# soopark0221/auction-gym

Measured on AMD Instinct MI355X. Metric: auctions resolved/sec (SP_Oracle-shaped batches), higher is better.
Workload: dtype f64

## Files before the change

### auction-gym_amd/csrc/ag_host.h

```cpp
#pragma once
#include <hip/hip_runtime.h>
#include <stdint.h>

#include "auctiongym.h"

int ag_set_error(int code, const char *fmt, ...) __attribute__((format(printf, 2, 3)));

#define AG_HIP(call)                                                                    \
  do {                                                                                  \
    hipError_t e_ = (call);                                                             \
    if (e_ != hipSuccess)                                                               \
      return ag_set_error(AG_ERR_HIP, "%s: %s (%s:%d)", #call, hipGetErrorString(e_),   \
                          __FILE__, __LINE__);                                          \
  } while (0)

template <typename T>
inline int ag_check_struct(const T *p, const char *who, const char *type) {
  if (p && p->struct_size != (uint64_t)sizeof(T))
    return ag_set_error(AG_ERR_INVALID,
                        "%s: %s.struct_size is %llu, this library (ABI %d) expects %llu -- the caller's "
                        "binding declares another layout of include/auctiongym.h",
                        who, type, (unsigned long long)p->struct_size, AG_ABI_VERSION,
                        (unsigned long long)sizeof(T));
  return AG_OK;
// ... 32 lines not shown
  uint32_t *key = nullptr;
  float *x = nullptr;
  int64_t *offsets = nullptr;
  double *adam_tab = nullptr;
  int32_t *epochs = nullptr;
  void *tables = nullptr;
  int64_t *partials = nullptr;
  size_t tables_bytes = 0, partials_bytes = 0;
  int coop_blocks = 0;
  struct {
    bool active = false;
    void *st = nullptr;
    void *acc = nullptr, *tables = nullptr;
    size_t st_bytes = 0, acc_bytes = 0, tables_bytes = 0;
    agtrain::RpAcc A{};
    agtrain::RpTables T{};
    int G = 0;
    int64_t k = 0;
    int64_t *totals = nullptr;
  } rp;
};

struct ag_dr_rp {
  bool active = false;
  void *st = nullptr;
  void *acc = nullptr, *tables = nullptr;
  size_t st_bytes = 0, acc_bytes = 0, tables_bytes = 0;
  agtrain::RpAcc A{};
  agtrain::RpTables T{};
  int G = 0, lines = 0;
  int64_t k = 0;
  int64_t *totals = nullptr;
  const float *noise = nullptr;
  int64_t noise_n = 0;
  int32_t noise_e0 = 0, noise_epochs = 0;
  agtrain::SortedRecs recs{};
  bool single = false;
  void *pipe = nullptr;
  size_t pipe_bytes = 0;
  void *pipe_st = nullptr;
  int pipe_blocks[2] = {0, 0};
};

struct ag_dr_ws {
  void *buf = nullptr;
  size_t buf_bytes = 0;
  int64_t *counts = nullptr;
  double *adam_tab = nullptr;
  float *state = nullptr;
  int32_t *init = nullptr;
  int32_t *mode = nullptr;
  int64_t *scratch = nullptr;
  void *coop = nullptr;
  size_t coop_bytes = 0;
  int coop_blocks = 0;
  int coop_blocks0 = 0;
  ag_dr_rp rp;
};

struct ag_ctx {
  int32_t device;
  ag_shape shape;
  int32_t D;
  int32_t item_search = AG_ITEM_SEARCH_AUTO;
  bool can_simulate = false;
  double *d_items = nullptr;
  double *d_values = nullptr;
  int64_t *d_partials = nullptr;
  uint32_t *d_queue = nullptr;
  int32_t partial_blocks = 0;
  int32_t resident[256] = {};
  bool ship_shape = true;
  bool gen_mode_all = false;
  int64_t launch_cap = 0;
  int64_t lrts_chunk = 0;
  bool wide = false;
  bool catalog = false;
  bool values_positive = false;
  bool ora_catalog = false;
  int32_t sim_kernel = AG_SIM_KERNEL_AUTO;
  int32_t grid_per_cu = 0;
  int32_t block_threads = 0;
  int32_t resident_slots[3][8] = {};
  int32_t resident_ora[8] = {};
  bool general = false, has_lrts = false, has_shading = false, lrts_loaded = false;
  int32_t ts_sample = 1;
  int32_t *h_akind = nullptr;
  int32_t *h_bkind = nullptr;
  bool dr_loaded = false, dr_any_init = false;
  bool vl_any_search = false;
  int64_t bidder_chunk = 0;
  int64_t bidder_cache = -1;
  uint64_t fit_noise_seed = 0;
  ag_dr_ws dr;
  int32_t *d_akind = nullptr, *d_bkind = nullptr;
  int32_t *d_kag = nullptr;
  bool ragged = false;
  double *d_pg = nullptr, *d_gs = nullptr;
  float *d_tsm = nullptr, *d_tsq = nullptr, *d_tsprev = nullptr;
  ag_lrts_ws lrts;
  int32_t *d_status = nullptr;
};

void ag_lrts_release(ag_ctx *c);
void ag_dr_release(ag_ctx *c);

inline int ag_one_slot_only(const ag_ctx *c, const char *who) {
  if (c && c->shape.num_slots > 1)
    return ag_set_error(AG_ERR_UNSUPPORTED, "%s: the context has num_slots = %d; rounds with several slots run "
                        "through ag_simulate_slots", who, c->shape.num_slots);
  return AG_OK;
}

inline int ag_check_store(const ag_ctx *c, const ag_lrts_samples *s, const char *who) {
  if (!c || !s) return ag_set_error(AG_ERR_INVALID, "%s: null argument", who);
  AG_CHECK_STRUCT(s, who, "ag_lrts_samples");
  if (!s->key || !s->x || !s->count || s->capacity < 0)
    return ag_set_error(AG_ERR_INVALID, "%s: sample store needs key, x, count and capacity >= 0", who);
  return AG_OK;
}
inline int ag_check_store(const ag_ctx *c, const ag_shading_samples *s, const char *who) {
  if (!c || !s) return ag_set_error(AG_ERR_INVALID, "%s: null argument", who);
  AG_CHECK_STRUCT(s, who, "ag_shading_samples");
  if (!s->agent || !s->gamma || !s->utility || !s->count || s->capacity < 0)
    return ag_set_error(AG_ERR_INVALID, "%s: sample store needs agent, gamma, utility, count, capacity", who);
  return AG_OK;
}

struct AgDeviceGuard {
  int prev = -1;
  explicit AgDeviceGuard(int dev) {
    if (hipGetDevice(&prev) == hipSuccess && prev != dev) (void)hipSetDevice(dev);
    else prev = -1;
  }
  ~AgDeviceGuard() {
    if (prev >= 0) (void)hipSetDevice(prev);
  }
};
```

### auction-gym_amd/csrc/ag_kernels.hip

```cpp
#include <hip/hip_runtime.h>

#include <math.h>
#include <stdarg.h>
#include <stdint.h>
#include <stdio.h>
#include <string.h>

#include <algorithm>
#include <string>

#include "ag_host.h"
#include "ag_philox.h"
#include "ag_sim.h"
#include "ag_sim_oracle.h"

static thread_local std::string g_last_error;

int ag_set_error(int code, const char *fmt, ...) {
  char buf[512];
  va_list ap;
  va_start(ap, fmt);
  vsnprintf(buf, sizeof buf, fmt, ap);
  va_end(ap);
  g_last_error = buf;
// ... 206 lines not shown
    s_v[threadIdx.x] = b < nb ? counts[b] : 0;
    __syncthreads();
    if (threadIdx.x == 0) {
      int64_t r = s_run;
      for (int t = 0; t < kThreads; ++t) {
        const int64_t c = s_v[t];
        s_v[t] = r;
        r += c;
      }
      s_run = r;
    }
    __syncthreads();
    if (b < nb) counts[b] = s_v[threadIdx.x];
    __syncthreads();
  }
  if (threadIdx.x == 0) counts[nb] = s_run;
}
__global__ __launch_bounds__(kThreads) void k_ts_index_write(const int32_t *part, const int32_t *akind, int64_t n,
                                                            const int64_t *offsets, int32_t *index) {
  __shared__ int s_w[kThreads / 64];
  const int64_t k0 = (int64_t)blockIdx.x * kScanTile + threadIdx.x * 4;
  int f[4], v = 0;
  for (int e = 0; e < 4; ++e) {
    f[e] = lrts_flag(part, akind, n, k0 + e);
    v += f[e];
  }
  int tot;
  int64_t r = offsets[blockIdx.x] + block_excl_scan(v, s_w, tot);
  for (int e = 0; e < 4; ++e)
    if (k0 + e < n) {
      index[k0 + e] = f[e] ? (int32_t)r : -1;
      r += f[e];
    }
}

__global__ __launch_bounds__(kThreads) void k_generate_grid(uint64_t seed, uint64_t first, int64_t B, int P,
                                                           double *grid) {
  const uint32_t k0 = (uint32_t)seed, k1 = (uint32_t)(seed >> 32);
  for (int64_t i = (int64_t)blockIdx.x * kThreads + threadIdx.x; i < B; i += (int64_t)gridDim.x * kThreads) {
    const uint64_t idx = first + (uint64_t)i;
    const uint32_t c0 = (uint32_t)idx, c1 = (uint32_t)(idx >> 32);
    for (int s = 0; s < P; ++s)
      for (int j = 0; j < 128; j += 2) {
        uint32_t w[4];
        philox(c0, c1, (uint32_t)(j >> 1), gen_stream(kDrawGrid, s), k0, k1, w);
        const double u0 = (double)((((uint64_t)w[0] << 32) | w[1]) >> 11) * 0x1p-53;
        const double u1 = (double)((((uint64_t)w[2] << 32) | w[3]) >> 11) * 0x1p-53;
        grid[((int64_t)s * 128 + j) * B + i] = 0.1 + 0.9 * u0;
        grid[((int64_t)s * 128 + j + 1) * B + i] = 0.1 + 0.9 * u1;
      }
  }
}

__global__ __launch_bounds__(kThreads) void k_exp_kat(const double *x, double *y, int64_t n, int sig) {
  __shared__ uint64_t s_tab[256];
  for (int i = threadIdx.x; i < 256; i += kThreads) s_tab[i] = ag_exp_tab[i];
  __syncthreads();
  for (int64_t i = (int64_t)blockIdx.x * kThreads + threadIdx.x; i < n; i += (int64_t)gridDim.x * kThreads)
    y[i] = sig ? agexp::sigmoid(x[i], s_tab) : agexp::exp(x[i], s_tab);
}

typedef uint32_t u32x4 __attribute__((ext_vector_type(4)));
__global__ __launch_bounds__(kThreads) void k_stream_copy(const u32x4 *__restrict__ src, u32x4 *__restrict__ dst,
                                                          int64_t n16) {
  const int64_t i = (int64_t)blockIdx.x * kThreads + threadIdx.x;
  if (i < n16) __builtin_nontemporal_store(__builtin_nontemporal_load(src + i), dst + i);
}

SimKernel pick_kernel(int P, int D, bool prune, int general, int bt) {
  if (P > kMaxP) return pick_kernel_for<0>(D, prune, general, bt);
  switch (P) {
    case 1: return pick_kernel_for<1>(D, prune, general, bt);
    case 2: return pick_kernel_for<2>(D, prune, general, bt);
    case 3: return pick_kernel_for<3>(D, prune, general, bt);
    case 4: return pick_kernel_for<4>(D, prune, general, bt);
    case 5: return pick_kernel_for<5>(D, prune, general, bt);
    case 6: return pick_kernel_for<6>(D, prune, general, bt);
    case 7: return pick_kernel_for<7>(D, prune, general, bt);
    case 8: return pick_kernel_for<8>(D, prune, general, bt);
    default: return nullptr;
  }
}

OraKernel pick_oracle(int P, int D, bool gen, uint32_t fields = 0, bool *spec = nullptr) {
  bool unused;
  if (!spec) spec = &unused;
  switch (P) {
    case 1: return pick_oracle_for<1>(D, gen, fields, spec);
    case 2: return pick_oracle_for<2>(D, gen, fields, spec);
    case 3: return pick_oracle_for<3>(D, gen, fields, spec);
    case 4: return pick_oracle_for<4>(D, gen, fields, spec);
    case 5: return pick_oracle_for<5>(D, gen, fields, spec);
    case 6: return pick_oracle_for<6>(D, gen, fields, spec);
    case 7: return pick_oracle_for<7>(D, gen, fields, spec);
    case 8: return pick_oracle_for<8>(D, gen, fields, spec);
    default: return nullptr;
  }
}

int resident_blocks(const ag_ctx *c, const void *k, size_t lds, int *out) {
  int per_cu = 0, cus = 0;
  AG_HIP(hipOccupancyMaxActiveBlocksPerMultiprocessor(&per_cu, k, kThreads, lds));
  AG_HIP(hipDeviceGetAttribute(&cus, hipDeviceAttributeMultiprocessorCount, c->device));
  int res = per_cu * cus;
  if (res < 1) res = 1;
  if (res > c->partial_blocks) res = c->partial_blocks;
  *out = res;
  return AG_OK;
}

int simulate_oracle(ag_ctx *c, int64_t B, const ag_batch_in *in, const ag_batch_out *out,
                    int64_t *counters_fx, hipStream_t st, uint64_t seed = 0, uint64_t first = 0) {
  const ag_shape &s = c->shape;
  OraParams prm;
  prm.B = (int32_t)B;
  prm.N = s.num_agents;
  prm.K = s.num_items;
  prm.mech = s.mechanism;
  prm.want_counters = counters_fx != nullptr;
  prm.L = make_ora_layout(s.num_agents, s.num_items, c->D, prm.want_counters);
  prm.items = c->d_items;
  prm.values = c->d_values;
  prm.ctx = in ? in->ctx : nullptr;
  prm.part = in ? in->part : nullptr;
  prm.u = in ? in->u : nullptr;
  prm.seed = seed;
  prm.first = first;
  prm.scale = s.embedding_var;
  prm.winner = out->winner;
  prm.price = out->price;
  prm.second_price = out->second_price;
  prm.outcome = out->outcome;
  prm.item = out->item;
  prm.bid = out->bid;
  prm.est_ctr = out->est_ctr;
  prm.true_ctr = out->true_ctr;
  prm.best_ev = out->best_ev;
  prm.winner_outcome = out->winner_outcome;
  prm.partials = c->d_partials;
  prm.queue = c->d_queue;
  bool is_spec = false;
  const OraKernel k = pick_oracle(s.num_participants, c->D, in == nullptr, ora_field_mask(prm), &is_spec);
  if (in && (int64_t)(c->D - 2) * B > (int64_t)UINT32_MAX)
    return ag_set_error(AG_ERR_UNSUPPORTED, "ag_simulate: (D - 2) * B must be < 2^32 (32-bit row offsets); "
                        "split the batch");
  const size_t lds = (size_t)prm.L.total;
  if (lds > 160 * 1024)
    return ag_set_error(AG_ERR_UNSUPPORTED, "ag_simulate: population needs %zu B of LDS (> 160 KiB)", lds);
  if (lds > 64 * 1024)
    AG_HIP(hipFuncSetAttribute((const void *)k, hipFuncAttributeMaxDynamicSharedMemorySize, (int)lds));
  int &res_max = c->resident_ora[(prm.want_counters ? 1 : 0) + (in ? 0 : 2) + (is_spec ? 4 : 0)];
  if (res_max == 0)
    if (int rc = resident_blocks(c, (const void *)k, lds, &res_max)) return rc;
  int res = res_max;
  {
    const int per_cu = c->grid_per_cu > 0 ? c->grid_per_cu : (is_spec ? kOraSpecBlocksPerCu : kOraBlocksPerCu);
    int cus = 0;
    AG_HIP(hipDeviceGetAttribute(&cus, hipDeviceAttributeMultiprocessorCount, c->device));
    if ((int64_t)per_cu * cus < res) res = per_cu * cus;
  }
  if (res >= 16) res &= ~15;
  int64_t chunk_max = (int64_t)res * kThreads * (ora_lane_cap(prm.L.replicas) / 2);
  prm.lane_tiles = (uint32_t)ora_lane_cap(prm.L.replicas);
  if (chunk_max > INT32_MAX) chunk_max = INT32_MAX;
  if (c->launch_cap > 0 && c->launch_cap < chunk_max) chunk_max = c->launch_cap;
  if (chunk_max < 1) chunk_max = 1;
  const int nc = s.num_agents * kC;
  for (int64_t lo = 0; lo < B; lo += chunk_max) {
    const int64_t hi = lo + chunk_max < B ? lo + chunk_max : B;
    const int64_t tiles = (hi - lo + kThreads - 1) / kThreads;
    int grid = (int)(tiles < res ? tiles : res);
    const int64_t chunks = (hi - lo + 64 * kOraChunkTiles - 1) / (64 * kOraChunkTiles);
    if (grid < 16 && chunks > 4 * (int64_t)grid) grid = (int)std::min<int64_t>(16, (chunks + 3) / 4);
    prm.lo = (int32_t)lo;
    prm.hi = (int32_t)hi;
    AG_HIP(hipMemsetAsync(c->d_queue, 0, sizeof(uint32_t) * 64 * 32, st));
    hipLaunchKernelGGL(k, dim3(grid), dim3(kThreads), lds, st, prm);
    AG_HIP(hipGetLastError());
    if (counters_fx) {
      hipLaunchKernelGGL(k_reduce_counters, dim3(nc), dim3(kThreads), 0, st, c->d_partials, grid, nc, counters_fx);
      AG_HIP(hipGetLastError());
    }
  }
  return AG_OK;
}

SimKernel pick_slots(int sm, int D, bool prune, int general) {
  switch (sm) {
    case 2: return pick_slots_for<2>(D, prune, general);
    case 4: return pick_slots_for<4>(D, prune, general);
    case 8: return pick_slots_for<8>(D, prune, general);
    default: return nullptr;
  }
}
int slots_build(int max_slots) { return max_slots <= 2 ? 2 : (max_slots <= 4 ? 4 : 8); }

int simulate_general(ag_ctx *c, int64_t B, const ag_batch_in *in, const ag_batch_out *out, int64_t *counters_fx,
                     hipStream_t st, bool gen, uint64_t seed, uint64_t first, const SlotsIo *sl = nullptr) {
  const ag_shape &s = c->shape;
  const int nc = s.num_agents * kC;
  const int D = c->D;
  const bool prune = c->item_search == AG_ITEM_SEARCH_AUTO && D <= 8 && s.num_items <= 2 * kMaxKPairs &&
                     c->values_positive;
  SimParams prm;
  prm.B = B;
  prm.N = s.num_agents;
  prm.K = s.num_items;
  prm.mech = s.mechanism;
  prm.want_counters = counters_fx != nullptr;
  prm.lds = make_layout(s.num_agents, s.num_items, D, prm.want_counters, c->general,
                        s.obs_embedding_size + 1, gen);
  prm.ts_sample = c->ts_sample;
  prm.akind = c->d_akind;
  prm.bkind = c->d_bkind;
  prm.pg = c->d_pg;
  prm.gs = c->d_gs;
  prm.tsm = c->d_tsm;
  prm.drs = c->dr_loaded ? c->dr.state : nullptr;
  prm.dri = c->dr_loaded ? c->dr.init : nullptr;
  prm.kag = c->ragged ? c->d_kag : nullptr;
  prm.items = c->d_items;
  prm.values = c->d_values;
  prm.in = in ? *in : ag_batch_in{};
  prm.out = *out;
  prm.partials = c->d_partials;
  prm.P = s.num_participants;
  prm.tsq = c->d_tsq;
  prm.seed = seed;
  prm.first = first;
  prm.scale = s.embedding_var;
  prm.sl = sl ? *sl : SlotsIo{};
  size_t lds = (size_t)prm.lds.total;
  if (lds > 160 * 1024)
    return ag_set_error(AG_ERR_UNSUPPORTED, "ag_simulate: population needs %zu B of LDS (> 160 KiB)", lds);
  int bt = c->block_threads;
  if (bt == 0) bt = (c->general && prune && lds > 40 * 1024) ? kLargeThreads : kThreads;
  if (sl) bt = kThreads;
  const int gmode = !c->general ? kGenOracle : (c->has_shading || c->gen_mode_all || sl) ? kGenAll : kGenTruthful;
  const int ship = (!sl && c->general && c->ship_shape && D == 6 && prm.lds.ts_do == kShipDo) ? kGenShip : 0;
  if (bt == kLargeThreads && c->block_threads == 0 && gmode == kGenAll && ship && s.num_participants >= AG_STREAM_MIN_P &&
      s.num_participants <= kMaxP)
    bt = kMidThreads;
  const int genb = gen ? kGenGen : 0;
  const int sm = sl ? slots_build(sl->max_slots) : 0;
  SimKernel k = sl ? pick_slots(sm, D, prune, gmode)
                   : pick_kernel(s.num_participants, D, prune, gmode | ship | genb, bt);
  if (sl && !k)
    return ag_set_error(AG_ERR_UNSUPPORTED, "ag_simulate_slots: supports E+1 in 2..8 (P=%d D=%d)",
                        s.num_participants, D);
  if (!k && bt == kMidThreads) {
    bt = kLargeThreads;
    k = pick_kernel(s.num_participants, D, prune, gmode | ship | genb, bt);
  }
  if (!k && !gen && c->general && c->block_threads == kLargeThreads)
    return ag_set_error(AG_ERR_UNSUPPORTED,
                        "ag_simulate: AG_OPT_SIM_BLOCK_THREADS = %d needs the screened item search (K <= %d, positive "
                        "catalogue values, E+1 <= 8) and P <= %d (P=%d D=%d K=%d)",
                        kLargeThreads, 2 * kMaxKPairs, kMaxP, s.num_participants, D, s.num_items);
  if (!k && bt != kThreads) {
    bt = kThreads;
// ... 654 lines not shown
```

### auction-gym_amd/csrc/ag_sim_oracle.h

```cpp
#pragma once
#include "ag_philox.h"
#include "ag_sim.h"

namespace ag {

constexpr int kOraSlotGross = 0, kOraSlotPaid = 1, kOraSlotUnderbid1 = 1, kOraSlotOverbid = 2,
              kOraSlotBestEv = 3, kOraSlotCounts = 4;
constexpr int kOraStride = 5;
constexpr double kOraMaxValue = 1024.0;
#ifndef AG_ORA_SPECIALISE
#define AG_ORA_SPECIALISE 1
#endif
constexpr int kOraFlush = 255;
constexpr int kOraChunkTiles = 8;
constexpr int kOraBlocksPerCu = 8;
constexpr int kOraSpecBlocksPerCu = 4;
__host__ inline int64_t ora_lane_cap(int R) { return 512 * (int64_t)R; }

struct OraLayout {
  int32_t tab, items, values, scr, scr_val, amax, cnt, total;
  int32_t items_stride, values_stride, scr_stride, scr_val_stride, kpairs, replicas;
};

__host__ inline OraLayout make_ora_layout(int N, int K, int D, bool counters) {
  OraLayout L;
  L.items_stride = (K * D) | 1;
  L.values_stride = K | 1;
  L.kpairs = (K + 1) / 2;
  L.scr_stride = L.kpairs * 16 + 4;
  L.scr_val_stride = L.kpairs * 2 + 2;
  int R = 64;
  while (R > 1 && (int64_t)N * R * kOraStride * 8 > 40960) R >>= 1;
  L.replicas = R;
  int64_t b = 256 * 8;
  L.tab = 0;
  L.items = align16(b);
  b = L.items + (int64_t)N * L.items_stride * 8;
  L.values = align16(b);
  b = L.values + (int64_t)N * L.values_stride * 8;
  L.scr = align16(b);
  b = L.scr + (int64_t)N * L.scr_stride * 4;
  L.scr_val = align16(b);
  b = L.scr_val + (int64_t)N * L.scr_val_stride * 4;
  L.amax = align16(b);
  b = L.amax + (int64_t)N * 4;
  L.cnt = align16(b);
  b = L.cnt + (counters ? (int64_t)N * R * kOraStride * 8 : 0);
  L.total = align16(b);
  return L;
}

struct OraParams {
  int32_t B;
  int32_t lo, hi;
  int32_t N, K, mech, want_counters;
  OraLayout L;
  const double *items, *values;
  const double *ctx;
  const int32_t *part;
  const double *u;
  int32_t *winner;
  double *price, *second_price;
  uint8_t *outcome;
  int32_t *item;
  double *bid, *est_ctr, *true_ctr, *best_ev;
  uint32_t *winner_outcome;
  int64_t *partials;
  uint32_t *queue;
  uint32_t lane_tiles;
  uint64_t seed, first;
  double scale;
};

constexpr uint32_t kOraFWinner = 1, kOraFPrice = 2, kOraFSecondPrice = 4, kOraFOutcome = 8, kOraFItem = 16,
                   kOraFBid = 32, kOraFEstCtr = 64, kOraFTrueCtr = 128, kOraFBestEv = 256, kOraFWinnerOutcome = 512;
constexpr uint32_t kOraHeadline =
    kOraFWinnerOutcome | kOraFPrice | kOraFItem | kOraFBid | kOraFEstCtr | kOraFTrueCtr | kOraFBestEv;
__host__ inline uint32_t ora_field_mask(const OraParams &p) {
  return (p.winner ? kOraFWinner : 0) | (p.price ? kOraFPrice : 0) | (p.second_price ? kOraFSecondPrice : 0) |
         (p.outcome ? kOraFOutcome : 0) | (p.item ? kOraFItem : 0) | (p.bid ? kOraFBid : 0) |
         (p.est_ctr ? kOraFEstCtr : 0) | (p.true_ctr ? kOraFTrueCtr : 0) | (p.best_ev ? kOraFBestEv : 0) |
         (p.winner_outcome ? kOraFWinnerOutcome : 0);
}
template <uint32_t FM, uint32_t BIT>
__device__ __forceinline__ bool ora_has(const void *p) {
  if constexpr (FM != 0) return (FM & BIT) != 0;
  else return p != nullptr;
}
__device__ __forceinline__ unsigned long long ora_fx(double x) {
  const double y = fma(x, kFxScale, kMagic);
  return (unsigned long long)(__double_as_longlong(y) - __double_as_longlong(kMagic));
}

template <int D>
__device__ __forceinline__ void ora_screen(const float *__restrict__ row, const float *__restrict__ sv, int kpairs,
                                           const float (&xf)[kMaxD], uint32_t &m1, uint32_t &m2) {
  m1 = 0xffffffffu;
  m2 = 0xffffffffu;
  for (int p = 0; p < kpairs; ++p) {
    const float *r = row + p * 16;
    f32x2 z = *reinterpret_cast<const f32x2 *>(r + 2 * (D - 1));
#pragma unroll
    for (int d = 0; d < D - 1; ++d) {
      const f32x2 a = *reinterpret_cast<const f32x2 *>(r + 2 * d);
      const f32x2 xd = {xf[d], xf[d]};
      z = __builtin_elementwise_fma(a, xd, z);
    }
    const f32x2 e = {__builtin_amdgcn_exp2f(z.x), __builtin_amdgcn_exp2f(z.y)};
    const f32x2 iv = *reinterpret_cast<const f32x2 *>(sv + 2 * p);
    const f32x2 t = __builtin_elementwise_fma(e, iv, iv);
    const uint32_t ta = (__float_as_uint(t.x) & ~15u) | (uint32_t)(2 * p);
    const uint32_t tb = (__float_as_uint(t.y) & ~15u) | (uint32_t)(2 * p + 1);
    const uint32_t lo = min(ta, tb), hi = max(ta, tb);
    m2 = min(min(max(m1, lo), m2), hi);
    m1 = min(m1, lo);
  }
}

template <int D>
__device__ __forceinline__ uint32_t ora_screen_one(const float *__restrict__ row, const float *__restrict__ sv,
                                                   int k, const float (&xf)[kMaxD]) {
  const float *r = row + (k >> 1) * 16 + (k & 1);
  float z = r[2 * (D - 1)];
#pragma unroll
  for (int d = 0; d < D - 1; ++d) z = fmaf(r[2 * d], xf[d], z);
  const float e = __builtin_amdgcn_exp2f(z);
  const float iv = sv[k];
  const float t = fmaf(e, iv, iv);
  return (__float_as_uint(t) & ~15u) | (uint32_t)k;
}

template <int P, int D, bool GEN, uint32_t FM = 0>
__global__ __launch_bounds__(kThreads) void k_oracle(OraParams prm) {
  extern __shared__ __attribute__((aligned(16))) unsigned char smem[];
  const int N = prm.N, K = prm.K;
  const uint32_t B = (uint32_t)prm.B, lo = (uint32_t)prm.lo, hi = (uint32_t)prm.hi;
  const OraLayout L = prm.L;
  uint64_t *s_tab = reinterpret_cast<uint64_t *>(smem + L.tab);
  double *s_items = reinterpret_cast<double *>(smem + L.items);
  double *s_vals = reinterpret_cast<double *>(smem + L.values);
  float *s_scr = reinterpret_cast<float *>(smem + L.scr);
  float *s_scr_val = reinterpret_cast<float *>(smem + L.scr_val);
  float *s_amax = reinterpret_cast<float *>(smem + L.amax);
  unsigned char *s_cnt = smem + L.cnt;

  const int tid = threadIdx.x;
  for (int i = tid; i < 256; i += kThreads) s_tab[i] = ag_exp_tab[i];
  for (int i = tid; i < N * K * D; i += kThreads) {
    const int a = i / (K * D), r = i - a * (K * D);
    s_items[a * L.items_stride + r] = prm.items[i];
  }
  for (int i = tid; i < N * K; i += kThreads) {
    const int a = i / K, r = i - a * K;
    s_vals[a * L.values_stride + r] = prm.values[i];
  }
  for (int i = tid; i < N * L.kpairs * 16; i += kThreads) {
    const int a = i / (L.kpairs * 16), r = i - a * (L.kpairs * 16);
    const int p = r >> 4, d = (r >> 1) & 7, k = 2 * p + (r & 1);
    const float c = (d < D && k < K) ? (float)prm.items[((size_t)a * K + k) * D + d] : 0.0f;
    s_scr[a * L.scr_stride + r] = c * kNegLog2e;
  }
  for (int i = tid; i < N * L.kpairs * 2; i += kThreads) {
    const int a = i / (L.kpairs * 2), k = i - a * (L.kpairs * 2);
    s_scr_val[a * L.scr_val_stride + k] = k < K ? 1.0f / (float)prm.values[(size_t)a * K + k] : INFINITY;
  }
  for (int a = tid; a < N; a += kThreads) {
    float m = 0.0f;
    for (int r = 0; r < K * D; ++r) m = fmaxf(m, (float)fabs(prm.items[(size_t)a * K * D + r]));
    s_amax[a] = m * 1.001f;
  }
  const int R = L.replicas;
  const int cnt_qwords = N * R * kOraStride;
  if (prm.want_counters)
    for (int i = tid; i < cnt_qwords; i += kThreads) reinterpret_cast<unsigned long long *>(s_cnt)[i] = 0ull;
  __syncthreads();

  const bool charged = P >= 2;
  const bool fp = prm.mech == AG_FIRST_PRICE;
  const bool packed = N <= 8;
  const uint32_t agent_bytes = (uint32_t)R * kOraStride * 8;
  const uint32_t lane_off = (uint32_t)(tid & (R - 1)) * kOraStride * 8;
  uint64_t n_logs_packed = 0, n_won_packed = 0;
  int since_flush = 0;
  auto cadd = [&](uint32_t addr, int slot, unsigned long long v) {
    atomicAdd(reinterpret_cast<unsigned long long *>(s_cnt + addr + slot * 8), v);
  };
  auto flush_counts = [&]() {
    for (int a = 0; a < N; ++a) {
      const uint64_t v = ((n_logs_packed >> (8 * a)) & 255ull) | (((n_won_packed >> (8 * a)) & 255ull) << 32);
      if (v) cadd((uint32_t)a * agent_bytes + lane_off, kOraSlotCounts, (unsigned long long)v);
    }
    n_logs_packed = 0;
    n_won_packed = 0;
    since_flush = 0;
  };

  const uint32_t q_lane = tid & 63;
  const uint32_t q_idx = ((uint32_t)blockIdx.x * (kThreads / 64) + (uint32_t)(tid >> 6)) & 63u;
  uint32_t *const q_ctr = prm.queue + q_idx * 32;
  constexpr uint32_t q_len = 64 * kOraChunkTiles;
  const uint32_t q_chunks = (hi - lo + q_len - 1) / q_len;
  uint32_t q_claims = 0;
  auto q_claim = [&]() -> uint32_t {
    uint32_t r = 0xffffffffu;
    if (q_claims < prm.lane_tiles / kOraChunkTiles) {
      if (q_lane == 0) r = atomicAdd(q_ctr, 1u);
      ++q_claims;
    }
    return r;
  };
  auto q_chunk_of = [&](uint32_t raw) -> uint32_t {
    const uint32_t t = (uint32_t)__builtin_amdgcn_readfirstlane((int)raw);
    return t == 0xffffffffu ? 0xffffffffu : t * 64u + q_idx;
  };
  uint32_t q_cur = q_chunk_of(q_claim());
  uint32_t q_raw = q_claim();
  while (q_cur < q_chunks) {
#pragma nounroll
    for (int q_s = 0; q_s < kOraChunkTiles; ++q_s) {
      const uint32_t i = lo + q_cur * q_len + (uint32_t)q_s * 64 + q_lane;
      if (i >= hi) break;
      auto at = [&](auto *base, uint32_t row) { return base + row + i; };
      double x[kMaxD];
      float xf[kMaxD];
      float xabs = 1.0f;
      int ag[P];
      double u;
      if constexpr (GEN) {
        gen_auction<P, kMaxD>((uint32_t)prm.seed, (uint32_t)(prm.seed >> 32), prm.first + i, N, P, D - 1,
                              prm.scale, x, ag, u);
      } else {
#pragma unroll
        for (int e = 0; e < D - 1; ++e) x[e] = ldg(at(prm.ctx, e * B));
#pragma unroll
        for (int s = 0; s < P; ++s) ag[s] = ldg(at(prm.part, s * B));
        u = ldg(at(prm.u, 0));
      }
#pragma unroll
      for (int e = 0; e < D - 1; ++e) {
        xf[e] = (float)x[e];
        xabs += fabsf(xf[e]);
      }
      x[D - 1] = 1.0;
      xf[D - 1] = 1.0f;
      xabs *= 1.001f;

      int w = 0;
      double m1 = 0.0, m2 = -INFINITY, ctr_w = 0.0, val_w = 0.0;
      double bevs[P];
      int itv[P];
      double bdv[P], ctv[P];
#pragma unroll
      for (int s = 0; s < P; ++s) {
        const int a = ag[s];
        const double *itm = s_items + a * L.items_stride;
        const double *vv = s_vals + a * L.values_stride;
        const float *row = s_scr + a * L.scr_stride;
        const float *sv = s_scr_val + a * L.scr_val_stride;
        uint32_t t1, t2;
        ora_screen<D>(row, sv, L.kpairs, xf, t1, t2);
        const bool ok = (s_amax[a] * xabs <= kPruneMaxS) && (__uint_as_float(t1 & ~15u) <= 1e30f);
        const float thr = __uint_as_float(t1 & ~15u) * (1.0f + kPruneDelta);
        int best = (int)(t1 & 15u);
        double c = agexp::sigmoid_fast(dot_ref<D>(itm + best * D, x), s_tab);
        double sc = c * vv[best];
        if (!ok || !(__uint_as_float(t2 & ~15u) > thr)) {
          const int kf = best;
          const double c_kf = c;
          best = -1;
          for (int k = 0; k < K; ++k) {
            if (ok && k != kf && !(__uint_as_float(ora_screen_one<D>(row, sv, k, xf) & ~15u) <= thr)) continue;
            const double ck = k == kf ? c_kf : agexp::sigmoid_fast(dot_ref<D>(itm + k * D, x), s_tab);
            const double sk = ck * vv[k];
            if (best < 0 || sk > sc || (sk == sc && k < best)) {
              best = k;
              sc = sk;
              c = ck;
            }
          }
        }
        const double v = vv[best];
        const double b = v * c;
        bevs[s] = sc;
        itv[s] = best;
        bdv[s] = b;
        ctv[s] = c;
        if (s == 0) {
          m1 = b;
          ctr_w = c;
          val_w = v;
        } else if (b > m1) {
          m2 = m1;
          m1 = b;
          w = s;
          ctr_w = c;
          val_w = v;
        } else if (b > m2) {
          m2 = b;
        }
      }
      const double price = fp ? m1 : m2;
      const int oc = bernoulli(ctr_w, u);
#pragma unroll
      for (int s = 0; s < P; ++s)
        if (ora_has<FM, kOraFItem>(prm.item)) stg(at(prm.item, s * B), (int32_t)itv[s]);
#pragma unroll
      for (int s = 0; s < P; ++s)
        if (ora_has<FM, kOraFBid>(prm.bid)) stg(at(prm.bid, s * B), bdv[s]);
#pragma unroll
      for (int s = 0; s < P; ++s)
        if (ora_has<FM, kOraFEstCtr>(prm.est_ctr)) stg(at(prm.est_ctr, s * B), ctv[s]);
#pragma unroll
      for (int s = 0; s < P; ++s)
        if (ora_has<FM, kOraFTrueCtr>(prm.true_ctr)) stg(at(prm.true_ctr, s * B), ctv[s]);
#pragma unroll
      for (int s = 0; s < P; ++s)
        if (ora_has<FM, kOraFBestEv>(prm.best_ev)) stg(at(prm.best_ev, s * B), bevs[s]);
      if (ora_has<FM, kOraFWinner>(prm.winner)) stg(at(prm.winner, 0), (int32_t)w);
      if (ora_has<FM, kOraFPrice>(prm.price)) stg(at(prm.price, 0), charged ? price : (double)NAN);
      if (ora_has<FM, kOraFSecondPrice>(prm.second_price)) stg(at(prm.second_price, 0), charged ? m2 : (double)NAN);
      if (ora_has<FM, kOraFOutcome>(prm.outcome)) stg(at(prm.outcome, 0), (uint8_t)oc);
      if (ora_has<FM, kOraFWinnerOutcome>(prm.winner_outcome)) stg(at(prm.winner_outcome, 0), pack_wo(w, oc));

      if (prm.want_counters) {
#pragma unroll
        for (int s = 0; s < P; ++s) {
          const uint32_t addr = (uint32_t)ag[s] * agent_bytes + lane_off;
          const bool won = charged && s == w;
          cadd(addr, kOraSlotBestEv, ora_fx(bevs[s]));
          if constexpr (P == 1) {
            if (bevs[s] > 0.0) cadd(addr, kOraSlotUnderbid1, ora_fx(-bevs[s]));
          }
          if (won) {
            cadd(addr, kOraSlotPaid, ora_fx(price));
            if (oc) cadd(addr, kOraSlotGross, ora_fx(val_w));
            if (fp && charged) {
              const unsigned long long ob = ora_fx(price - m2);
              if (ob) cadd(addr, kOraSlotOverbid, ob);
            }
          }
          if (packed) {
            const uint64_t bit = 1ull << (8 * ag[s]);
            n_logs_packed += bit;
            if (won) n_won_packed += bit;
          } else {
            cadd(addr, kOraSlotCounts, won ? 0x100000001ull : 1ull);
          }
        }
        if (packed && ++since_flush == kOraFlush) flush_counts();
      }
    }
    q_cur = q_chunk_of(q_raw);
    q_raw = q_claim();
  }

  if (!prm.want_counters) return;
  if (packed) flush_counts();
  __syncthreads();
  unsigned long long *cnt = reinterpret_cast<unsigned long long *>(s_cnt);
  auto split = [&](int j, unsigned long long c, long long &l, long long &h) {
    if (j == kOraSlotCounts) {
      l = (long long)(c & 0xffffffffull);
      h = (long long)(c >> 32);
    } else {
      l = (long long)c & kLimbMask;
      h = (long long)c >> AG_FX_LIMB_BITS;
    }
  };
  if (R >= 2) {
    for (int pr = tid; pr < N * kOraStride; pr += kThreads) {
      const int a = pr / kOraStride, j = pr - a * kOraStride;
      const unsigned long long *c0 = cnt + (size_t)a * R * kOraStride + j;
      long long sl = 0, sh = 0;
      for (int r0 = 0; r0 < R; r0 += 8) {
        unsigned long long v[8];
#pragma unroll
        for (int u = 0; u < 8; ++u) v[u] = r0 + u < R ? c0[(size_t)(r0 + u) * kOraStride] : 0ull;
#pragma unroll
        for (int u = 0; u < 8; ++u) {
          long long l, h;
          split(j, v[u], l, h);
          sl += l;
          sh += h;
        }
      }
      cnt[(size_t)a * R * kOraStride + j] = (unsigned long long)sl;
      cnt[((size_t)a * R + 1) * kOraStride + j] = (unsigned long long)sh;
    }
    __syncthreads();
  }
  for (int a = tid; a < N; a += kThreads) {
    long long lo_[kOraStride], hi_[kOraStride];
    for (int j = 0; j < kOraStride; ++j) {
      if (R >= 2) {
        lo_[j] = (long long)cnt[(size_t)a * R * kOraStride + j];
        hi_[j] = (long long)cnt[((size_t)a * R + 1) * kOraStride + j];
      } else {
        split(j, cnt[(size_t)a * kOraStride + j], lo_[j], hi_[j]);
      }
    }
    int64_t *dst = prm.partials + ((size_t)blockIdx.x * N + a) * kC * 2;
    auto put = [&](int c, long long l, long long h) {
      dst[2 * c] = l;
      dst[2 * c + 1] = h;
    };
    auto put_count = [&](int c, unsigned long long n) {
      put(c, (long long)((n & 63ull) << AG_FX_FRAC_BITS), (long long)(n >> 6));
    };
    const unsigned long long nlogs = (unsigned long long)lo_[kOraSlotCounts];
    const unsigned long long nwon = (unsigned long long)hi_[kOraSlotCounts];
    if constexpr (P == 1)
      put(AG_C_NET, lo_[kOraSlotGross], hi_[kOraSlotGross]);
    else
      put(AG_C_NET, lo_[kOraSlotGross] - lo_[kOraSlotPaid], hi_[kOraSlotGross] - hi_[kOraSlotPaid]);
    put(AG_C_GROSS, lo_[kOraSlotGross], hi_[kOraSlotGross]);
    put(AG_C_ALLOC_REGRET, 0, 0);
    put(AG_C_EST_REGRET, 0, 0);
    put(AG_C_OVERBID, lo_[kOraSlotOverbid], hi_[kOraSlotOverbid]);
    if constexpr (P == 1)
      put(AG_C_UNDERBID, lo_[kOraSlotUnderbid1], hi_[kOraSlotUnderbid1]);
    else
      put(AG_C_UNDERBID, 0, 0);
    put(AG_C_CTR_SQERR, 0, 0);
    put_count(AG_C_CTR_BIAS, nwon);
    put(AG_C_BEST_EV, lo_[kOraSlotBestEv], hi_[kOraSlotBestEv]);
    put_count(AG_C_N_LOGS, nlogs);
    put_count(AG_C_N_WON, nwon);
    if constexpr (P == 1)
      put(AG_C_PAID, 0, 0);
    else
      put(AG_C_PAID, lo_[kOraSlotPaid], hi_[kOraSlotPaid]);
  }
}

typedef void (*OraKernel)(OraParams);

template <int P>
OraKernel pick_oracle_for(int D, bool gen, uint32_t fields, bool *spec);
template <> OraKernel pick_oracle_for<0>(int, bool, uint32_t, bool *);
template <> OraKernel pick_oracle_for<1>(int, bool, uint32_t, bool *);
template <> OraKernel pick_oracle_for<2>(int, bool, uint32_t, bool *);
template <> OraKernel pick_oracle_for<3>(int, bool, uint32_t, bool *);
template <> OraKernel pick_oracle_for<4>(int, bool, uint32_t, bool *);
template <> OraKernel pick_oracle_for<5>(int, bool, uint32_t, bool *);
template <> OraKernel pick_oracle_for<6>(int, bool, uint32_t, bool *);
template <> OraKernel pick_oracle_for<7>(int, bool, uint32_t, bool *);
template <> OraKernel pick_oracle_for<8>(int, bool, uint32_t, bool *);

}
```

### auction-gym_amd/csrc/ag_sim_p.hip

```cpp
#include "ag_sim.h"
#include "ag_sim_oracle.h"

#ifndef AG_P
#error "compile with -DAG_P=<participants>"
#endif

namespace ag {
namespace {

template <int P, bool PRUNE, int G, int BT = kThreads>
SimKernel pick_d(int D) {
  switch (D) {
    case 2: return k_simulate<P, 2, PRUNE, G, BT>;
    case 3: return k_simulate<P, 3, PRUNE, G, BT>;
    case 4: return k_simulate<P, 4, PRUNE, G, BT>;
    case 5: return k_simulate<P, 5, PRUNE, G, BT>;
    case 6: return k_simulate<P, 6, PRUNE, G, BT>;
    case 7: return k_simulate<P, 7, PRUNE, G, BT>;
    case 8: return k_simulate<P, 8, PRUNE, G, BT>;
    default: return nullptr;
  }
}

}

#if AG_P == 0
template <>
SimKernel pick_kernel_for<0>(int D, bool prune, int general, int bt) {
  if (general & kGenGen) return nullptr;
  general &= ~kGenShip;
  if (bt != kThreads || D > 8) return nullptr;
  if (general) return prune ? pick_d<0, true, kGenAll>(D) : pick_d<0, false, kGenAll>(D);
  return prune ? pick_d<0, true, kGenOracle>(D) : pick_d<0, false, kGenOracle>(D);
}

template <>
OraKernel pick_oracle_for<0>(int, bool, uint32_t, bool *spec) {
  *spec = false;
  return nullptr;
}
#else
template <>
SimKernel pick_kernel_for<AG_P>(int D, bool prune, int general, int bt) {
  constexpr int P = AG_P;
  const bool ship = (general & kGenShip) != 0;
  const bool genm = (general & kGenGen) != 0;
  general &= ~(kGenShip | kGenGen);
  if (genm) {
    if (!general || !ship || !prune || D != 6) return nullptr;
    if (bt == kLargeThreads) return k_simulate<P, 6, true, kGenAll, kLargeThreads, kShipDo, true>;
    if constexpr (P >= AG_STREAM_MIN_P)
      if (bt == kMidThreads && general == kGenAll) return k_simulate<P, 6, true, kGenAll, kMidThreads, kShipDo, true>;
    if (bt != kThreads) return nullptr;
    if (general == kGenTruthful) return k_simulate<P, 6, true, kGenTruthful, kThreads, kShipDo, true>;
    return k_simulate<P, 6, true, kGenAll, kThreads, kShipDo, true>;
  }
  if (general && ship && prune && D == 6) {
    if (bt == kLargeThreads) return k_simulate<P, 6, true, kGenAll, kLargeThreads, kShipDo>;
    if constexpr (P >= AG_STREAM_MIN_P)
      if (bt == kMidThreads && general == kGenAll) return k_simulate<P, 6, true, kGenAll, kMidThreads, kShipDo>;
    if (bt != kThreads) return nullptr;
    if (general == kGenTruthful) return k_simulate<P, 6, true, kGenTruthful, kThreads, kShipDo>;
    return k_simulate<P, 6, true, kGenAll, kThreads, kShipDo>;
  }
  if (general) {
    if (D > 8) return nullptr;
    if (bt == kLargeThreads) return prune ? pick_d<P, true, kGenAll, kLargeThreads>(D) : nullptr;
    if (bt != kThreads) return nullptr;
    if (general == kGenTruthful)
      return prune ? pick_d<P, true, kGenTruthful>(D) : pick_d<P, false, kGenTruthful>(D);
    return prune ? pick_d<P, true, kGenAll>(D) : pick_d<P, false, kGenAll>(D);
  }
  if (bt != kThreads) return nullptr;
  if (prune) return pick_d<P, true, kGenOracle>(D);
  if (D <= 8) return pick_d<P, false, kGenOracle>(D);
  switch (D) {
    case 9: return k_simulate<P, 9, false, kGenOracle>;
    case 11: return k_simulate<P, 11, false, kGenOracle>;
    case 13: return k_simulate<P, 13, false, kGenOracle>;
    case 16: return k_simulate<P, 16, false, kGenOracle>;
    default: return nullptr;
  }
}

template <>
OraKernel pick_oracle_for<AG_P>(int D, bool gen, uint32_t fields, bool *spec) {
  constexpr int P = AG_P;
  *spec = false;
#if AG_ORA_SPECIALISE
  if (D == 6 && fields == kOraHeadline) {
    *spec = true;
    return gen ? k_oracle<P, 6, true, kOraHeadline> : k_oracle<P, 6, false, kOraHeadline>;
  }
#endif
  switch (D) {
    case 2: return gen ? k_oracle<P, 2, true> : k_oracle<P, 2, false>;
    case 3: return gen ? k_oracle<P, 3, true> : k_oracle<P, 3, false>;
    case 4: return gen ? k_oracle<P, 4, true> : k_oracle<P, 4, false>;
    case 5: return gen ? k_oracle<P, 5, true> : k_oracle<P, 5, false>;
    case 6: return gen ? k_oracle<P, 6, true> : k_oracle<P, 6, false>;
    case 7: return gen ? k_oracle<P, 7, true> : k_oracle<P, 7, false>;
    case 8: return gen ? k_oracle<P, 8, true> : k_oracle<P, 8, false>;
    default: return nullptr;
  }
}
#endif

}
```

Baseline: 36.90 billion.

## Add paired-auction oracle kernel with 16-byte vector loads and stores

Adds a PAIR variant of the oracle kernel for P=2, D=6 headline fields on HBM inputs. Each lane resolves two adjacent auctions and uses 2-wide vector loads and stores for contexts, participants, u and the outputs. The host picks it only when pointers are aligned, the batch and range bounds are even, and residency is no worse than the base kernel. The aim is fewer and wider memory transactions, paid for with more registers per thread and an extra kernel instantiation.

```diff
diff --git a/auction-gym_amd/csrc/ag_host.h b/auction-gym_amd/csrc/ag_host.h
--- a/auction-gym_amd/csrc/ag_host.h
+++ b/auction-gym_amd/csrc/ag_host.h
@@ -138,7 +138,7 @@
   int32_t grid_per_cu = 0;
   int32_t block_threads = 0;
   int32_t resident_slots[3][8] = {};
-  int32_t resident_ora[8] = {};
+  int32_t resident_ora[10] = {};
   bool general = false, has_lrts = false, has_shading = false, lrts_loaded = false;
   int32_t ts_sample = 1;
   int32_t *h_akind = nullptr;
diff --git a/auction-gym_amd/csrc/ag_kernels.hip b/auction-gym_amd/csrc/ag_kernels.hip
--- a/auction-gym_amd/csrc/ag_kernels.hip
+++ b/auction-gym_amd/csrc/ag_kernels.hip
@@ -312,18 +312,18 @@
   }
 }
 
-OraKernel pick_oracle(int P, int D, bool gen, uint32_t fields = 0, bool *spec = nullptr) {
+OraKernel pick_oracle(int P, int D, bool gen, uint32_t fields = 0, bool *spec = nullptr, bool pair = false) {
   bool unused;
   if (!spec) spec = &unused;
   switch (P) {
-    case 1: return pick_oracle_for<1>(D, gen, fields, spec);
-    case 2: return pick_oracle_for<2>(D, gen, fields, spec);
-    case 3: return pick_oracle_for<3>(D, gen, fields, spec);
-    case 4: return pick_oracle_for<4>(D, gen, fields, spec);
-    case 5: return pick_oracle_for<5>(D, gen, fields, spec);
-    case 6: return pick_oracle_for<6>(D, gen, fields, spec);
-    case 7: return pick_oracle_for<7>(D, gen, fields, spec);
-    case 8: return pick_oracle_for<8>(D, gen, fields, spec);
+    case 1: return pick_oracle_for<1>(D, gen, fields, pair, spec);
+    case 2: return pick_oracle_for<2>(D, gen, fields, pair, spec);
+    case 3: return pick_oracle_for<3>(D, gen, fields, pair, spec);
+    case 4: return pick_oracle_for<4>(D, gen, fields, pair, spec);
+    case 5: return pick_oracle_for<5>(D, gen, fields, pair, spec);
+    case 6: return pick_oracle_for<6>(D, gen, fields, pair, spec);
+    case 7: return pick_oracle_for<7>(D, gen, fields, pair, spec);
+    case 8: return pick_oracle_for<8>(D, gen, fields, pair, spec);
     default: return nullptr;
   }
 }
@@ -382,6 +382,21 @@
   int &res_max = c->resident_ora[(prm.want_counters ? 1 : 0) + (in ? 0 : 2) + (is_spec ? 4 : 0)];
   if (res_max == 0)
     if (int rc = resident_blocks(c, (const void *)k, lds, &res_max)) return rc;
+  const OraKernel k_pair = pick_oracle(s.num_participants, c->D, in == nullptr, ora_field_mask(prm), nullptr, true);
+  auto aligned = [](const void *p, uintptr_t a) { return (reinterpret_cast<uintptr_t>(p) & (a - 1)) == 0; };
+  const bool pair_ok = k_pair != k && in && B % 2 == 0 && aligned(prm.ctx, 16) && aligned(prm.u, 16) &&
+                       aligned(prm.price, 16) && aligned(prm.bid, 16) && aligned(prm.est_ctr, 16) &&
+                       aligned(prm.true_ctr, 16) && aligned(prm.best_ev, 16) && aligned(prm.part, 8) &&
+                       aligned(prm.item, 8) && aligned(prm.winner_outcome, 8);
+  int res_pair = 0;
+  if (pair_ok) {
+    if (lds > 64 * 1024)
+      AG_HIP(hipFuncSetAttribute((const void *)k_pair, hipFuncAttributeMaxDynamicSharedMemorySize, (int)lds));
+    int &rp = c->resident_ora[8 + (prm.want_counters ? 1 : 0)];
+    if (rp == 0)
+      if (int rc = resident_blocks(c, (const void *)k_pair, lds, &rp)) return rc;
+    res_pair = rp;
+  }
   int res = res_max;
   {
     const int per_cu = c->grid_per_cu > 0 ? c->grid_per_cu : (is_spec ? kOraSpecBlocksPerCu : kOraBlocksPerCu);
@@ -404,8 +419,9 @@
     if (grid < 16 && chunks > 4 * (int64_t)grid) grid = (int)std::min<int64_t>(16, (chunks + 3) / 4);
     prm.lo = (int32_t)lo;
     prm.hi = (int32_t)hi;
+    const bool pair = pair_ok && lo % 2 == 0 && hi % 2 == 0 && res_pair >= res;
     AG_HIP(hipMemsetAsync(c->d_queue, 0, sizeof(uint32_t) * 64 * 32, st));
-    hipLaunchKernelGGL(k, dim3(grid), dim3(kThreads), lds, st, prm);
+    hipLaunchKernelGGL(pair ? k_pair : k, dim3(grid), dim3(kThreads), lds, st, prm);
     AG_HIP(hipGetLastError());
     if (counters_fx) {
       hipLaunchKernelGGL(k_reduce_counters, dim3(nc), dim3(kThreads), 0, st, c->d_partials, grid, nc, counters_fx);
diff --git a/auction-gym_amd/csrc/ag_sim_oracle.h b/auction-gym_amd/csrc/ag_sim_oracle.h
--- a/auction-gym_amd/csrc/ag_sim_oracle.h
+++ b/auction-gym_amd/csrc/ag_sim_oracle.h
@@ -1,4 +1,6 @@
 #pragma once
+#include <type_traits>
+
 #include "ag_philox.h"
 #include "ag_sim.h"
 
@@ -10,6 +12,9 @@
 constexpr double kOraMaxValue = 1024.0;
 #ifndef AG_ORA_SPECIALISE
 #define AG_ORA_SPECIALISE 1
+#endif
+#ifndef AG_ORA_PAIR
+#define AG_ORA_PAIR 1
 #endif
 constexpr int kOraFlush = 255;
 constexpr int kOraChunkTiles = 8;
@@ -130,7 +135,18 @@
   return (__float_as_uint(t) & ~15u) | (uint32_t)k;
 }
 
-template <int P, int D, bool GEN, uint32_t FM = 0>
+typedef double f64x2 __attribute__((ext_vector_type(2)));
+typedef int32_t i32x2 __attribute__((ext_vector_type(2)));
+
+template <int P>
+struct OraRes {
+  double bevs[P], bdv[P], ctv[P];
+  int itv[P];
+  int w, oc;
+  double price, m2, val_w;
+};
+
+template <int P, int D, bool GEN, uint32_t FM = 0, bool PAIR = false>
 __global__ __launch_bounds__(kThreads) void k_oracle(OraParams prm) {
   extern __shared__ __attribute__((aligned(16))) unsigned char smem[];
   const int N = prm.N, K = prm.K;
@@ -213,141 +229,198 @@
     const uint32_t t = (uint32_t)__builtin_amdgcn_readfirstlane((int)raw);
     return t == 0xffffffffu ? 0xffffffffu : t * 64u + q_idx;
   };
+  auto resolve = [&](double (&x)[kMaxD], const int (&ag)[P], double u, OraRes<P> &r) __attribute__((always_inline)) {
+    float xf[kMaxD];
+    float xabs = 1.0f;
+#pragma unroll
+    for (int e = 0; e < D - 1; ++e) {
+      xf[e] = (float)x[e];
+      xabs += fabsf(xf[e]);
+    }
+    x[D - 1] = 1.0;
+    xf[D - 1] = 1.0f;
+    xabs *= 1.001f;
+
+    int w = 0;
+    double m1 = 0.0, m2 = -INFINITY, ctr_w = 0.0, val_w = 0.0;
+#pragma unroll
+    for (int s = 0; s < P; ++s) {
+      const int a = ag[s];
+      const double *itm = s_items + a * L.items_stride;
+      const double *vv = s_vals + a * L.values_stride;
+      const float *row = s_scr + a * L.scr_stride;
+      const float *sv = s_scr_val + a * L.scr_val_stride;
+      uint32_t t1, t2;
+      ora_screen<D>(row, sv, L.kpairs, xf, t1, t2);
+      const bool ok = (s_amax[a] * xabs <= kPruneMaxS) && (__uint_as_float(t1 & ~15u) <= 1e30f);
+      const float thr = __uint_as_float(t1 & ~15u) * (1.0f + kPruneDelta);
+      int best = (int)(t1 & 15u);
+      double c = agexp::sigmoid_fast(dot_ref<D>(itm + best * D, x), s_tab);
+      double sc = c * vv[best];
+      if (!ok || !(__uint_as_float(t2 & ~15u) > thr)) {
+        const int kf = best;
+        const double c_kf = c;
+        best = -1;
+        for (int k = 0; k < K; ++k) {
+          if (ok && k != kf && !(__uint_as_float(ora_screen_one<D>(row, sv, k, xf) & ~15u) <= thr)) continue;
+          const double ck = k == kf ? c_kf : agexp::sigmoid_fast(dot_ref<D>(itm + k * D, x), s_tab);
+          const double sk = ck * vv[k];
+          if (best < 0 || sk > sc || (sk == sc && k < best)) {
+            best = k;
+            sc = sk;
+            c = ck;
+          }
+        }
+      }
+      const double v = vv[best];
+      const double b = v * c;
+      r.bevs[s] = sc;
+      r.itv[s] = best;
+      r.bdv[s] = b;
+      r.ctv[s] = c;
+      if (s == 0) {
+        m1 = b;
+        ctr_w = c;
+        val_w = v;
+      } else if (b > m1) {
+        m2 = m1;
+        m1 = b;
+        w = s;
+        ctr_w = c;
+        val_w = v;
+      } else if (b > m2) {
+        m2 = b;
+      }
+    }
+    r.w = w;
+    r.m2 = m2;
+    r.val_w = val_w;
+    r.price = fp ? m1 : m2;
+    r.oc = bernoulli(ctr_w, u);
+  };
+  auto count = [&](const int (&ag)[P], const OraRes<P> &r) __attribute__((always_inline)) {
+    if (!prm.want_counters) return;
+#pragma unroll
+    for (int s = 0; s < P; ++s) {
+      const uint32_t addr = (uint32_t)ag[s] * agent_bytes + lane_off;
+      const bool won = charged && s == r.w;
+      cadd(addr, kOraSlotBestEv, ora_fx(r.bevs[s]));
+      if constexpr (P == 1) {
+        if (r.bevs[s] > 0.0) cadd(addr, kOraSlotUnderbid1, ora_fx(-r.bevs[s]));
+      }
+      if (won) {
+        cadd(addr, kOraSlotPaid, ora_fx(r.price));
+        if (r.oc) cadd(addr, kOraSlotGross, ora_fx(r.val_w));
+        if (fp && charged) {
+          const unsigned long long ob = ora_fx(r.price - r.m2);
+          if (ob) cadd(addr, kOraSlotOverbid, ob);
+        }
+      }
+      if (packed) {
+        const uint64_t bit = 1ull << (8 * ag[s]);
+        n_logs_packed += bit;
+        if (won) n_won_packed += bit;
+      } else {
+        cadd(addr, kOraSlotCounts, won ? 0x100000001ull : 1ull);
+      }
+    }
+    if (packed && ++since_flush == kOraFlush) flush_counts();
+  };
+
   uint32_t q_cur = q_chunk_of(q_claim());
   uint32_t q_raw = q_claim();
   while (q_cur < q_chunks) {
+    if constexpr (PAIR) {
+      static_assert(!PAIR || (!GEN && FM == kOraHeadline), "the pair form stores the headline's set from HBM inputs");
+      static_assert(kOraChunkTiles % 2 == 0, "a chunk is a whole number of pair-tiles");
 #pragma nounroll
-    for (int q_s = 0; q_s < kOraChunkTiles; ++q_s) {
-      const uint32_t i = lo + q_cur * q_len + (uint32_t)q_s * 64 + q_lane;
-      if (i >= hi) break;
-      auto at = [&](auto *base, uint32_t row) { return base + row + i; };
-      double x[kMaxD];
-      float xf[kMaxD];
-      float xabs = 1.0f;
-      int ag[P];
-      double u;
-      if constexpr (GEN) {
-        gen_auction<P, kMaxD>((uint32_t)prm.seed, (uint32_t)(prm.seed >> 32), prm.first + i, N, P, D - 1,
-                              prm.scale, x, ag, u);
-      } else {
-#pragma unroll
-        for (int e = 0; e < D - 1; ++e) x[e] = ldg(at(prm.ctx, e * B));
-#pragma unroll
-        for (int s = 0; s < P; ++s) ag[s] = ldg(at(prm.part, s * B));
-        u = ldg(at(prm.u, 0));
-      }
-#pragma unroll
-      for (int e = 0; e < D - 1; ++e) {
-        xf[e] = (float)x[e];
-        xabs += fabsf(xf[e]);
-      }
-      x[D - 1] = 1.0;
-      xf[D - 1] = 1.0f;
-      xabs *= 1.001f;
-
-      int w = 0;
-      double m1 = 0.0, m2 = -INFINITY, ctr_w = 0.0, val_w = 0.0;
-      double bevs[P];
-      int itv[P];
-      double bdv[P], ctv[P];
-#pragma unroll
-      for (int s = 0; s < P; ++s) {
-        const int a = ag[s];
-        const double *itm = s_items + a * L.items_stride;
-        const double *vv = s_vals + a * L.values_stride;
-        const float *row = s_scr + a * L.scr_stride;
-        const float *sv = s_scr_val + a * L.scr_val_stride;
-        uint32_t t1, t2;
-        ora_screen<D>(row, sv, L.kpairs, xf, t1, t2);
-        const bool ok = (s_amax[a] * xabs <= kPruneMaxS) && (__uint_as_float(t1 & ~15u) <= 1e30f);
-        const float thr = __uint_as_float(t1 & ~15u) * (1.0f + kPruneDelta);
-        int best = (int)(t1 & 15u);
-        double c = agexp::sigmoid_fast(dot_ref<D>(itm + best * D, x), s_tab);
-        double sc = c * vv[best];
-        if (!ok || !(__uint_as_float(t2 & ~15u) > thr)) {
-          const int kf = best;
-          const double c_kf = c;
-          best = -1;
-          for (int k = 0; k < K; ++k) {
-            if (ok && k != kf && !(__uint_as_float(ora_screen_one<D>(row, sv, k, xf) & ~15u) <= thr)) continue;
-            const double ck = k == kf ? c_kf : agexp::sigmoid_fast(dot_ref<D>(itm + k * D, x), s_tab);
-            const double sk = ck * vv[k];
-            if (best < 0 || sk > sc || (sk == sc && k < best)) {
-              best = k;
-              sc = sk;
-              c = ck;
-            }
-          }
+      for (int q_s = 0; q_s < kOraChunkTiles / 2; ++q_s) {
+        const uint32_t i = lo + q_cur * q_len + (uint32_t)q_s * 128 + 2 * q_lane;
+        if (i >= hi) break;
+        auto ld2 = [&](auto v, const auto *base, uint32_t row) {
+          return ldg(reinterpret_cast<const decltype(v) *>(base + row + i));
+        };
+        f64x2 xv[D - 1];
+        i32x2 av[P];
+#pragma unroll
+        for (int e = 0; e < D - 1; ++e) xv[e] = ld2(f64x2{}, prm.ctx, e * B);
+#pragma unroll
+        for (int s = 0; s < P; ++s) av[s] = ld2(i32x2{}, prm.part, s * B);
+        const f64x2 uv = ld2(f64x2{}, prm.u, 0);
+        OraRes<P> r0, r1;
+        auto half = [&](auto h, OraRes<P> &r) __attribute__((always_inline)) {
+          constexpr int H = decltype(h)::value;
+          double x[kMaxD];
+          int ag[P];
+#pragma unroll
+          for (int e = 0; e < D - 1; ++e) x[e] = xv[e][H];
+#pragma unroll
+          for (int s = 0; s < P; ++s) ag[s] = av[s][H];
+          resolve(x, ag, uv[H], r);
+          count(ag, r);
+        };
+        half(std::integral_constant<int, 0>{}, r0);
+        half(std::integral_constant<int, 1>{}, r1);
+        auto st2 = [&](auto *base, uint32_t row, auto a, auto b) {
+          typedef decltype(a) __attribute__((ext_vector_type(2))) V2;
+          stg(reinterpret_cast<V2 *>(base + row + i), V2{a, b});
+        };
+#pragma unroll
+        for (int s = 0; s < P; ++s) st2(prm.item, s * B, (int32_t)r0.itv[s], (int32_t)r1.itv[s]);
+#pragma unroll
+        for (int s = 0; s < P; ++s) st2(prm.bid, s * B, r0.bdv[s], r1.bdv[s]);
+#pragma unroll
+        for (int s = 0; s < P; ++s) st2(prm.est_ctr, s * B, r0.ctv[s], r1.ctv[s]);
+#pragma unroll
+        for (int s = 0; s < P; ++s) st2(prm.true_ctr, s * B, r0.ctv[s], r1.ctv[s]);
+#pragma unroll
+        for (int s = 0; s < P; ++s) st2(prm.best_ev, s * B, r0.bevs[s], r1.bevs[s]);
+        st2(prm.price, 0, charged ? r0.price : (double)NAN, charged ? r1.price : (double)NAN);
+        st2(prm.winner_outcome, 0, pack_wo(r0.w, r0.oc), pack_wo(r1.w, r1.oc));
+      }
+    } else {
+#pragma nounroll
+      for (int q_s = 0; q_s < kOraChunkTiles; ++q_s) {
+        const uint32_t i = lo + q_cur * q_len + (uint32_t)q_s * 64 + q_lane;
+        if (i >= hi) break;
+        auto at = [&](auto *base, uint32_t row) { return base + row + i; };
+        double x[kMaxD];
+        int ag[P];
+        double u;
+        if constexpr (GEN) {
+          gen_auction<P, kMaxD>((uint32_t)prm.seed, (uint32_t)(prm.seed >> 32), prm.first + i, N, P, D - 1,
+                                prm.scale, x, ag, u);
+        } else {
+#pragma unroll
+          for (int e = 0; e < D - 1; ++e) x[e] = ldg(at(prm.ctx, e * B));
+#pragma unroll
+          for (int s = 0; s < P; ++s) ag[s] = ldg(at(prm.part, s * B));
+          u = ldg(at(prm.u, 0));
         }
-        const double v = vv[best];
-        const double b = v * c;
-        bevs[s] = sc;
-        itv[s] = best;
-        bdv[s] = b;
-        ctv[s] = c;
-        if (s == 0) {
-          m1 = b;
-          ctr_w = c;
-          val_w = v;
-        } else if (b > m1) {
-          m2 = m1;
-          m1 = b;
-          w = s;
-          ctr_w = c;
-          val_w = v;
-        } else if (b > m2) {
-          m2 = b;
-        }
-      }
-      const double price = fp ? m1 : m2;
-      const int oc = bernoulli(ctr_w, u);
-#pragma unroll
-      for (int s = 0; s < P; ++s)
-        if (ora_has<FM, kOraFItem>(prm.item)) stg(at(prm.item, s * B), (int32_t)itv[s]);
-#pragma unroll
-      for (int s = 0; s < P; ++s)
-        if (ora_has<FM, kOraFBid>(prm.bid)) stg(at(prm.bid, s * B), bdv[s]);
-#pragma unroll
-      for (int s = 0; s < P; ++s)
-        if (ora_has<FM, kOraFEstCtr>(prm.est_ctr)) stg(at(prm.est_ctr, s * B), ctv[s]);
-#pragma unroll
-      for (int s = 0; s < P; ++s)
-        if (ora_has<FM, kOraFTrueCtr>(prm.true_ctr)) stg(at(prm.true_ctr, s * B), ctv[s]);
-#pragma unroll
-      for (int s = 0; s < P; ++s)
-        if (ora_has<FM, kOraFBestEv>(prm.best_ev)) stg(at(prm.best_ev, s * B), bevs[s]);
-      if (ora_has<FM, kOraFWinner>(prm.winner)) stg(at(prm.winner, 0), (int32_t)w);
-      if (ora_has<FM, kOraFPrice>(prm.price)) stg(at(prm.price, 0), charged ? price : (double)NAN);
-      if (ora_has<FM, kOraFSecondPrice>(prm.second_price)) stg(at(prm.second_price, 0), charged ? m2 : (double)NAN);
-      if (ora_has<FM, kOraFOutcome>(prm.outcome)) stg(at(prm.outcome, 0), (uint8_t)oc);
-      if (ora_has<FM, kOraFWinnerOutcome>(prm.winner_outcome)) stg(at(prm.winner_outcome, 0), pack_wo(w, oc));
-
-      if (prm.want_counters) {
-#pragma unroll
-        for (int s = 0; s < P; ++s) {
-          const uint32_t addr = (uint32_t)ag[s] * agent_bytes + lane_off;
-          const bool won = charged && s == w;
-          cadd(addr, kOraSlotBestEv, ora_fx(bevs[s]));
-          if constexpr (P == 1) {
-            if (bevs[s] > 0.0) cadd(addr, kOraSlotUnderbid1, ora_fx(-bevs[s]));
-          }
-          if (won) {
-            cadd(addr, kOraSlotPaid, ora_fx(price));
-            if (oc) cadd(addr, kOraSlotGross, ora_fx(val_w));
-            if (fp && charged) {
-              const unsigned long long ob = ora_fx(price - m2);
-              if (ob) cadd(addr, kOraSlotOverbid, ob);
-            }
-          }
-          if (packed) {
-            const uint64_t bit = 1ull << (8 * ag[s]);
-            n_logs_packed += bit;
-            if (won) n_won_packed += bit;
-          } else {
-            cadd(addr, kOraSlotCounts, won ? 0x100000001ull : 1ull);
-          }
-        }
-        if (packed && ++since_flush == kOraFlush) flush_counts();
+        OraRes<P> r;
+        resolve(x, ag, u, r);
+#pragma unroll
+        for (int s = 0; s < P; ++s)
+          if (ora_has<FM, kOraFItem>(prm.item)) stg(at(prm.item, s * B), (int32_t)r.itv[s]);
+#pragma unroll
+        for (int s = 0; s < P; ++s)
+          if (ora_has<FM, kOraFBid>(prm.bid)) stg(at(prm.bid, s * B), r.bdv[s]);
+#pragma unroll
+        for (int s = 0; s < P; ++s)
+          if (ora_has<FM, kOraFEstCtr>(prm.est_ctr)) stg(at(prm.est_ctr, s * B), r.ctv[s]);
+#pragma unroll
+        for (int s = 0; s < P; ++s)
+          if (ora_has<FM, kOraFTrueCtr>(prm.true_ctr)) stg(at(prm.true_ctr, s * B), r.ctv[s]);
+#pragma unroll
+        for (int s = 0; s < P; ++s)
+          if (ora_has<FM, kOraFBestEv>(prm.best_ev)) stg(at(prm.best_ev, s * B), r.bevs[s]);
+        if (ora_has<FM, kOraFWinner>(prm.winner)) stg(at(prm.winner, 0), (int32_t)r.w);
+        if (ora_has<FM, kOraFPrice>(prm.price)) stg(at(prm.price, 0), charged ? r.price : (double)NAN);
+        if (ora_has<FM, kOraFSecondPrice>(prm.second_price))
+          stg(at(prm.second_price, 0), charged ? r.m2 : (double)NAN);
+        if (ora_has<FM, kOraFOutcome>(prm.outcome)) stg(at(prm.outcome, 0), (uint8_t)r.oc);
+        if (ora_has<FM, kOraFWinnerOutcome>(prm.winner_outcome)) stg(at(prm.winner_outcome, 0), pack_wo(r.w, r.oc));
+        count(ag, r);
       }
     }
     q_cur = q_chunk_of(q_raw);
@@ -436,15 +509,15 @@
 typedef void (*OraKernel)(OraParams);
 
 template <int P>
-OraKernel pick_oracle_for(int D, bool gen, uint32_t fields, bool *spec);
-template <> OraKernel pick_oracle_for<0>(int, bool, uint32_t, bool *);
-template <> OraKernel pick_oracle_for<1>(int, bool, uint32_t, bool *);
-template <> OraKernel pick_oracle_for<2>(int, bool, uint32_t, bool *);
-template <> OraKernel pick_oracle_for<3>(int, bool, uint32_t, bool *);
-template <> OraKernel pick_oracle_for<4>(int, bool, uint32_t, bool *);
-template <> OraKernel pick_oracle_for<5>(int, bool, uint32_t, bool *);
-template <> OraKernel pick_oracle_for<6>(int, bool, uint32_t, bool *);
-template <> OraKernel pick_oracle_for<7>(int, bool, uint32_t, bool *);
-template <> OraKernel pick_oracle_for<8>(int, bool, uint32_t, bool *);
-
-}
+OraKernel pick_oracle_for(int D, bool gen, uint32_t fields, bool pair, bool *spec);
+template <> OraKernel pick_oracle_for<0>(int, bool, uint32_t, bool, bool *);
+template <> OraKernel pick_oracle_for<1>(int, bool, uint32_t, bool, bool *);
+template <> OraKernel pick_oracle_for<2>(int, bool, uint32_t, bool, bool *);
+template <> OraKernel pick_oracle_for<3>(int, bool, uint32_t, bool, bool *);
+template <> OraKernel pick_oracle_for<4>(int, bool, uint32_t, bool, bool *);
+template <> OraKernel pick_oracle_for<5>(int, bool, uint32_t, bool, bool *);
+template <> OraKernel pick_oracle_for<6>(int, bool, uint32_t, bool, bool *);
+template <> OraKernel pick_oracle_for<7>(int, bool, uint32_t, bool, bool *);
+template <> OraKernel pick_oracle_for<8>(int, bool, uint32_t, bool, bool *);
+
+}
diff --git a/auction-gym_amd/csrc/ag_sim_p.hip b/auction-gym_amd/csrc/ag_sim_p.hip
--- a/auction-gym_amd/csrc/ag_sim_p.hip
+++ b/auction-gym_amd/csrc/ag_sim_p.hip
@@ -35,7 +35,7 @@
 }
 
 template <>
-OraKernel pick_oracle_for<0>(int, bool, uint32_t, bool *spec) {
+OraKernel pick_oracle_for<0>(int, bool, uint32_t, bool, bool *spec) {
   *spec = false;
   return nullptr;
 }
@@ -84,12 +84,15 @@
 }
 
 template <>
-OraKernel pick_oracle_for<AG_P>(int D, bool gen, uint32_t fields, bool *spec) {
+OraKernel pick_oracle_for<AG_P>(int D, bool gen, uint32_t fields, bool pair, bool *spec) {
   constexpr int P = AG_P;
   *spec = false;
 #if AG_ORA_SPECIALISE
   if (D == 6 && fields == kOraHeadline) {
     *spec = true;
+#if AG_P == 2 && AG_ORA_PAIR
+    if (pair && !gen) return k_oracle<P, 6, false, kOraHeadline, true>;
+#endif
     return gen ? k_oracle<P, 6, true, kOraHeadline> : k_oracle<P, 6, false, kOraHeadline>;
   }
 #endif
```

Result: slower. 36.34 billion (-1.5%).
